# NLAFET/preAlps

Hardware: AMD Instinct MI355X
Metric: ECG iters/sec + SpMM HBM GB/s (% roofline), 3D-elasticity n~1M t=4 (higher is better)
Workload: dtype f64; 1 GPU; Q1 3-D elasticity, 70^3 nodes, the reference's element matrix (nu=0.25), stiff/soft inclusions (examples/test_ecg_petsc_ela.c:217-347) (N=1029000, nnz=80990208), ECG odir + block-Jacobi, t=4, tol 1e-5; nparts=5670, partition=boxes of [2, 4, 8] nodes, parallelism=rows x1, comm=none, hip_graphs=False, bj_max_bandwidth=35, spmm_blocks=4174

## Files before the change

### prealps_amd/csrc/bj_priv.h

```cpp
#ifndef PA_BJ_PRIV_H
#define PA_BJ_PRIV_H

#include "pa_host.h"
#include "bj_build.h"
#include "coarse_space.h"

typedef struct {
  int on;
  int k, naggr, nc, nchunks, n;
  double* V;
  int* part_aggregate;
  double* d_zv; int* d_ch_row0; int* d_ch_nrows; int* d_ch_aggr; int* d_agg_ptr; int* d_agg_chunk;
  double* d_Einv; double* d_partial; double* d_c; double* d_y;
  pa_coarse_plan_t plan;
  double bytes, setup_s;
  int builds; long long applies;
} pa_bj_coarse_t;

typedef struct {
  int created;
  pa_bj_coarse_t co;
  int np;
  int m;
  int* d_row0; int* d_nrows; int* d_bw; long long* d_off;
  int* d_map_f; int* d_map_b;
  double* d_Lf; double* d_Lb; double* d_invd_f; double* d_invd_b;
  double* d_Lf2; double* d_Lb2; long long* d_off2;
  double pairs_bytes;
  void* d_Lg4; int g4_bits; double g4_bytes;
  int* d_class_list[PA_BJ_MAX_CLASSES];
  const int* class_list_c[PA_BJ_MAX_CLASSES];
  pa_bj_plan_t plan;
  double factor_bytes; int nd_blocks;
  pa_bj_layout_t lay;
  int* h_row0; int* h_nrows; int* h_bw; int* h_grow0; int* h_map_f; char* h_is_nd;
  int row_off, dev_factor, dev_wmax, nd_bits;
  const int* A_rowptr;
  int op_build;
  unsigned* d_bm_src; unsigned* d_bm_dst; int* d_bm_chunk_blk; unsigned* d_bm_chunk_first;
  size_t bm_n, bm_nchunks, bm_bytes;
  long long* d_boff; int* d_slist; int* d_blist; int* d_fail;
  int bm_builds, updates, nd_rebuilt;
  double upd_map_s, upd_copy_s, upd_kernel_s, upd_total_s;
} pa_bj_t;

pa_bj_t* pa_bj_state(void);
void pa_bj_apply_epoch_bump(void);
void pa_bj_values_epoch_sync(void);
int pa_bj_factor_launch(const pa_bj_t* s, const int* d_slist, const int* d_blist, const long long* d_boff,
                        double* d_band, int* d_fail, int* fail);
int pa_bj_fail_global_row(int row_off, const int* map_f, const int* row0, const int* nrows, int np, int fail);
int pa_bj_nd_handoff(const char* who, const CPLM_Mat_CSR_t* A, int np, const char* is_nd, int nnd, const int* row0,
                     const int* nrows, const int* grow0, int m, int bits, int row_off);
int pa_bj_launch_g4(const pa_bj_t* s);
int pa_bj_launch_pairs(const pa_bj_t* s);

void pa_bj_coarse_release(pa_bj_coarse_t* co);
int pa_bj_coarse_refresh(pa_bj_t* s, const pa_operator_info_t* op);

#endif
```

### prealps_amd/csrc/bj_refactor.hip

```cpp
#include "kernels_common.h"

namespace {

__global__ __launch_bounds__(WG) void k_bj_band_assemble(const unsigned* __restrict__ src, const unsigned* __restrict__ dst,
                                                        const int* __restrict__ chunk_blk,
                                                        const unsigned* __restrict__ chunk_first, int nchunks,
                                                        const long long* __restrict__ boff,
                                                        const double* __restrict__ pv, double* __restrict__ band) {
  for (int c = blockIdx.x; c < nchunks; c += gridDim.x) {
    const unsigned e0 = chunk_first[c], e1 = chunk_first[c + 1];
    double* __restrict__ out = band + boff[chunk_blk[c]];
    for (unsigned base = e0 + threadIdx.x; base < e1; base += 4 * WG) {
      unsigned s[4], d[4];
      double v[4];
#pragma unroll
      for (int u = 0; u < 4; ++u) {
        const unsigned e = base + u * WG;
        s[u] = e < e1 ? __builtin_nontemporal_load(src + e) : 0u;
        d[u] = e < e1 ? __builtin_nontemporal_load(dst + e) : 0u;
      }
#pragma unroll
      for (int u = 0; u < 4; ++u) v[u] = base + u * WG < e1 ? pv[s[u]] : 0.0;
#pragma unroll
      for (int u = 0; u < 4; ++u) if (base + u * WG < e1) out[d[u]] = v[u];
    }
  }
}

}

extern "C" int pa_k_bj_band_assemble(const unsigned* src, const unsigned* dst, const int* chunk_blk,
                                     const unsigned* chunk_first, size_t nchunks, const long long* boff,
                                     const double* pv, double* band) {
  if (nchunks == 0) return 0;
  if (nchunks > 0x7fffffffu) { pa_rt_set_error("k_bj_band_assemble: %zu chunks", nchunks); return 1; }
  const int cus = pa_rt_num_cus() > 0 ? pa_rt_num_cus() : 256;
  size_t blocks = nchunks;
  if (blocks > (size_t)8 * cus) blocks = (size_t)8 * cus;
  PA_LAUNCH(k_bj_band_assemble, dim3((unsigned)blocks), dim3(WG), 0, cur_stream(), src, dst, chunk_blk, chunk_first,
            (int)nchunks, boff, pv, band);
  return kfail("k_bj_band_assemble");
}
```

### prealps_amd/csrc/bj_update.c

```c
#include <stdio.h>
#include <stdlib.h>
#include <string.h>

#include "bj_priv.h"

#define BJU_FAIL(...) pa_fail_at("preAlps_BlockJacobiUpdateValues", __VA_ARGS__)

static void bj_band_map_release(pa_bj_t* s) {
  pa_rt_free(s->d_bm_src); pa_rt_free(s->d_bm_dst); pa_rt_free(s->d_bm_chunk_blk); pa_rt_free(s->d_bm_chunk_first);
  pa_rt_free(s->d_boff); pa_rt_free(s->d_slist); pa_rt_free(s->d_blist); pa_rt_free(s->d_fail);
  s->d_bm_src = s->d_bm_dst = s->d_bm_chunk_first = NULL; s->d_bm_chunk_blk = s->d_slist = s->d_blist = s->d_fail = NULL;
  s->d_boff = NULL;
}

static int bj_ensure_band_map(pa_bj_t* s, const pa_operator_info_t* op) {
  if (s->d_bm_src) return 0;
  const int np = s->np;
  const pa_bj_layout_t* L = &s->lay;
  const double t0 = pa_wtime();
  pa_bj_band_map_in_t in = {.np = np, .rowPtr = op->A.rowPtr, .colInd = op->A.colInd, .row0 = s->h_row0, .nrows = s->h_nrows,
                            .grow0 = s->h_grow0, .bw = s->h_bw, .order = s->h_map_f, .is_nd = s->h_is_nd,
                            .wmax = s->dev_wmax, .chunk = 1024};
  pa_bj_band_map_t bm;
  const int brc = pa_bj_band_map_build(&in, &bm);
  if (brc == -2)
    return BJU_FAIL("the band of block %d (%d rows, bandwidth %d) has 2^32 entries or more: free and create instead",
                    bm.bad_block, s->h_nrows[bm.bad_block], s->h_bw[bm.bad_block]);
  if (brc == -3) return BJU_FAIL("block %d of the panel no longer has the pattern the preconditioner was created from", bm.bad_block);
  if (brc) return BJU_FAIL("out of host memory for the band map");
  ++s->bm_builds;
  int rc = 0;
  s->d_bm_src = (unsigned*)pa_rt_malloc((bm.n ? bm.n : 1) * sizeof(unsigned));
  s->d_bm_dst = (unsigned*)pa_rt_malloc((bm.n ? bm.n : 1) * sizeof(unsigned));
  s->d_bm_chunk_blk = (int*)pa_rt_malloc((bm.nchunks ? bm.nchunks : 1) * sizeof(int));
  s->d_bm_chunk_first = (unsigned*)pa_rt_malloc((bm.nchunks + 1) * sizeof(unsigned));
  s->d_boff = (long long*)pa_rt_malloc(((size_t)np + 1) * sizeof(long long));
  s->d_slist = (int*)pa_rt_malloc((L->ns ? L->ns : 1) * sizeof(int));
  s->d_blist = (int*)pa_rt_malloc((L->nbig ? L->nbig : 1) * sizeof(int));
  s->d_fail = (int*)pa_rt_malloc(sizeof(int));
  if (!s->d_bm_src || !s->d_bm_dst || !s->d_bm_chunk_blk || !s->d_bm_chunk_first || !s->d_boff || !s->d_slist ||
      !s->d_blist || !s->d_fail ||
      pa_rt_h2d(s->d_bm_src, bm.src, bm.n * sizeof(unsigned)) || pa_rt_h2d(s->d_bm_dst, bm.dst, bm.n * sizeof(unsigned)) ||
      pa_rt_h2d(s->d_bm_chunk_blk, bm.chunk_blk, bm.nchunks * sizeof(int)) ||
      pa_rt_h2d(s->d_bm_chunk_first, bm.chunk_first, (bm.nchunks + 1) * sizeof(unsigned)) ||
      pa_rt_h2d(s->d_boff, L->boff, ((size_t)np + 1) * sizeof(long long)) ||
      pa_rt_h2d(s->d_slist, L->slist, (size_t)L->ns * sizeof(int)) || pa_rt_h2d(s->d_blist, L->blist, (size_t)L->nbig * sizeof(int))) {
    rc = BJU_FAIL("uploading the band map (%zu entries) failed: %s", bm.n, pa_rt_error());
    bj_band_map_release(s);
  }
  if (!rc) {
    s->bm_n = bm.n; s->bm_nchunks = bm.nchunks; s->bm_bytes = pa_bj_band_map_bytes(&bm);
    s->upd_map_s = pa_wtime() - t0;
  }
  pa_bj_band_map_free(&bm);
  return rc;
}

static int bj_refactor_bands(pa_bj_t* s, const pa_operator_info_t* op, int* wrote, int* spd_fail) {
  const size_t lnnz = (size_t)op->A.rowPtr[s->m], btot = s->lay.btot;
  double* d_pv = (double*)pa_rt_malloc((lnnz ? lnnz : 1) * sizeof(double));
  double* d_band = (double*)pa_rt_malloc((btot ? btot : 1) * sizeof(double));
  void* e0 = pa_rt_event_create();
  void* e1 = pa_rt_event_create();
  int rc = 0, fail = 0;
  if (!d_pv || !d_band || !e0 || !e1)
    rc = BJU_FAIL("no device memory for the panel values (%zu) and the bands (%zu entries): %s", lnnz, btot, pa_rt_error());
  if (!rc) {
    const double t0 = pa_wtime();
    if (pa_rt_h2d(d_pv, op->A.val, lnnz * sizeof(double))) rc = BJU_FAIL("uploading the panel values failed: %s", pa_rt_error());
    s->upd_copy_s = pa_wtime() - t0;
  }
  if (!rc) {
    *wrote = 1;
    if (pa_rt_event_record(e0) || pa_rt_memset(d_band, 0, btot * sizeof(double)) || pa_rt_memset(s->d_fail, 0, sizeof(int)) ||
        pa_k_bj_band_assemble(s->d_bm_src, s->d_bm_dst, s->d_bm_chunk_blk, s->d_bm_chunk_first, s->bm_nchunks, s->d_boff,
                              d_pv, d_band) ||
        pa_bj_factor_launch(s, s->d_slist, s->d_blist, s->d_boff, d_band, s->d_fail, &fail))
      rc = BJU_FAIL("factorising the diagonal blocks on the device failed: %s", pa_rt_error());
    *spd_fail = fail;
  }
  if (!rc && fail == 0) {
    if (s->d_Lg4 && pa_bj_launch_g4(s)) rc = BJU_FAIL("k_bj_g4_setup failed");
    if (!rc && s->d_Lf2 && pa_bj_launch_pairs(s)) rc = BJU_FAIL("k_bj_pairs failed");
    if (!rc && (pa_rt_event_record(e1) || pa_rt_sync())) rc = BJU_FAIL("%s", pa_rt_error());
    if (!rc) s->upd_kernel_s = pa_rt_event_elapsed_s(e0, e1);
  }
  pa_rt_event_destroy(e0); pa_rt_event_destroy(e1);
  pa_rt_free(d_pv); pa_rt_free(d_band);
  return rc;
}

int preAlps_BlockJacobiUpdateValues(void) {
  pa_bj_t* s = pa_bj_state();
  const double t_all = pa_wtime();
  if (!s->created) return BJU_FAIL("preconditioner not created");
  const pa_operator_info_t* op = pa_operator_info();
  if (!op) return BJU_FAIL("operator not built: it was freed since preAlps_BlockJacobiCreate (free and create instead)");
  if (pa_operator_build_count() != s->op_build)
    return BJU_FAIL("the operator was built again since preAlps_BlockJacobiCreate: free and create instead");
  if (s->A_rowptr != op->A.rowPtr)
    return BJU_FAIL("the preconditioner was not created from the operator's own panel (preAlps_OperatorGetA): free and create instead");
  if (!s->dev_factor)
    return BJU_FAIL("the preconditioner was created with PREALPS_BJ_FACTOR=host, its records come from the host "
                    "Cholesky: free and create instead");
  int rc = 0, wrote = 0, spd_fail = 0;
  s->upd_copy_s = s->upd_kernel_s = 0.0;
  if (s->np - s->nd_blocks > 0) {
    rc = bj_ensure_band_map(s, op);
    if (rc) return rc;
    rc = bj_refactor_bands(s, op, &wrote, &spd_fail);
    if (!rc && spd_fail > 0)
      rc = BJU_FAIL("diagonal block is not SPD (global row %d)",
                    pa_bj_fail_global_row(s->row_off, s->h_map_f, s->h_row0, s->h_nrows, s->np, spd_fail));
    if (rc && !wrote) return rc;
  }
  if (!rc && s->nd_blocks > 0) {
    rc = pa_bj_nd_handoff("preAlps_BlockJacobiUpdateValues", &op->A, s->np, s->h_is_nd, s->nd_blocks, s->h_row0, s->h_nrows,
                          s->h_grow0, s->m, s->nd_bits, s->row_off);
    if (!rc) { s->nd_rebuilt = s->nd_blocks; s->factor_bytes = 2.0 * 8.0 * (double)s->lay.tot + pa_nd_factor_bytes(); }
  }
  if (rc) { preAlps_BlockJacobiFree(); return rc; }
  ++s->updates;
  pa_bj_values_epoch_sync();
  if (s->co.on) rc = pa_bj_coarse_refresh(s, op);
  s->upd_total_s = pa_wtime() - t_all;
  return rc;
}

int pa_bj_update_stat(const char* key, double* value) {
  const pa_bj_t* s = pa_bj_state();
  const int on = s->created;
  if (!strcmp(key, "bj_updates")) *value = on ? s->updates : 0;
  else if (!strcmp(key, "bj_update_nd_rebuilt")) *value = on ? s->nd_rebuilt : 0;
  else if (!strcmp(key, "bj_band_map_builds")) *value = on ? s->bm_builds : 0;
  else if (!strcmp(key, "bj_band_map_entries")) *value = on && s->d_bm_src ? (double)s->bm_n : 0.0;
  else if (!strcmp(key, "bj_band_map_bytes")) *value = on && s->d_bm_src ? (double)s->bm_bytes : 0.0;
  else if (!strcmp(key, "bj_update_map_s")) *value = on ? s->upd_map_s : 0.0;
  else if (!strcmp(key, "bj_update_copy_s")) *value = on ? s->upd_copy_s : 0.0;
  else if (!strcmp(key, "bj_update_kernel_s")) *value = on ? s->upd_kernel_s : 0.0;
  else if (!strcmp(key, "bj_update_total_s")) *value = on ? s->upd_total_s : 0.0;
  else if (!strcmp(key, "bj_records_address")) *value = on ? (double)(size_t)s->d_Lf : 0.0;
  else if (!strcmp(key, "bj_g4_address")) *value = on ? (double)(size_t)s->d_Lg4 : 0.0;
  else if (!strcmp(key, "bj_coarse_max_dofs")) *value = PA_COARSE_MAX_DOFS;
  else if (!strncmp(key, "bj_coarse_", 10)) {
    const pa_bj_coarse_t* co = &s->co;
    const int con = on && co->on;
    const char* sub = key + 10;
    if (!strcmp(sub, "dofs")) *value = con ? co->nc : 0;
    else if (!strcmp(sub, "vectors")) *value = con ? co->k : 0;
    else if (!strcmp(sub, "aggregates")) *value = con ? co->naggr : 0;
    else if (!strcmp(sub, "chunks")) *value = con ? co->nchunks : 0;
    else if (!strcmp(sub, "bytes")) *value = con ? co->bytes : 0.0;
    else if (!strcmp(sub, "setup_s")) *value = con ? co->setup_s : 0.0;
    else if (!strcmp(sub, "builds")) *value = con ? co->builds : 0;
    else if (!strcmp(sub, "applies")) *value = con ? (double)co->applies : 0.0;
    else if (!strcmp(sub, "einv_address")) *value = con ? (double)(size_t)co->d_Einv : 0.0;
    else return 1;
  }
  else return 1;
  return 0;
}
```

### prealps_amd/csrc/block_jacobi.c

```c
#include <stdio.h>
#include <stdlib.h>
#include <string.h>

#include "bj_priv.h"

static pa_bj_t g_bj;
pa_bj_t* pa_bj_state(void) { return &g_bj; }
static double g_bj_setup_s[2];
double pa_bj_setup_seconds(int which) { return g_bj_setup_s[which ? 1 : 0]; }

double pa_bj_factor_bytes(void) { return g_bj.created ? g_bj.factor_bytes : 0.0; }
static int g_bj_values_epoch;
int pa_bj_values_epoch(void) { return g_bj_values_epoch; }
void pa_bj_values_epoch_sync(void) { g_bj_values_epoch = pa_operator_values_epoch(); }
int pa_bj_max_bandwidth(void) { return g_bj.created ? g_bj.lay.max_bw : 0; }
int pa_bj_nparts(void) { return g_bj.created ? g_bj.np : 0; }
int pa_bj_nd_blocks(void) { return g_bj.created ? g_bj.nd_blocks : 0; }
int pa_bj_nd_precision(void) { return g_bj.created && g_bj.nd_blocks > 0 ? pa_nd_precision() : 0; }

static int g_nd_bits = 0;
int preAlps_hip_set_nd_precision(int bits) {
  if (bits != 0 && bits != 32 && bits != 64)
    return PA_FAIL("precision %d refused: 64 (double), 32 (single) or 0 (follow PREALPS_BJ_ND_PRECISION)", bits);
  g_nd_bits = bits;
  return 0;
}
int pa_bj_band_precision(void) { return g_bj.created && g_bj.d_Lg4 ? g_bj.g4_bits : 0; }

static int g_band_bits = 0;
int preAlps_hip_set_band_precision(int bits) {
  if (bits != 0 && bits != 32 && bits != 64)
    return PA_FAIL("precision %d refused: 64 (double), 32 (single) or 0 (follow PREALPS_BJ_BAND_PRECISION)", bits);
  g_band_bits = bits;
  return 0;
}
double pa_bj_pairs_bytes(void) { return g_bj.created ? g_bj.pairs_bytes : 0.0; }
double pa_bj_g4_bytes(void) { return g_bj.created ? g_bj.g4_bytes : 0.0; }
int pa_bj_gram_blocks(void) {
  const pa_bj_t* s = &g_bj;
  const pa_bj_layout_t* L = &s->lay;
  if (!s->created || s->nd_blocks > 0 || !s->d_Lg4 || L->nclass != 1 || !L->class_g4[0] || L->class_count[0] != s->np) return 0;
  if (s->co.on) return 0;
  return s->np;
}

static int g_bj_apply_epoch;
int pa_bj_apply_epoch(void) { return g_bj_apply_epoch; }
void pa_bj_apply_epoch_bump(void) { ++g_bj_apply_epoch; }

void preAlps_BlockJacobiFree(void) {
  pa_bj_t* s = &g_bj;
  pa_bj_coarse_release(&s->co);
  ++g_bj_apply_epoch;
  pa_rt_free(s->d_row0); pa_rt_free(s->d_nrows); pa_rt_free(s->d_bw); pa_rt_free(s->d_off);
  pa_rt_free(s->d_map_f); pa_rt_free(s->d_map_b);
  pa_rt_free(s->d_Lf); pa_rt_free(s->d_Lb); pa_rt_free(s->d_invd_f); pa_rt_free(s->d_invd_b);
  pa_rt_free(s->d_Lf2); pa_rt_free(s->d_Lb2); pa_rt_free(s->d_off2); pa_rt_free(s->d_Lg4);
  for (int c = 0; c < PA_BJ_MAX_CLASSES; ++c) pa_rt_free(s->d_class_list[c]);
  pa_bj_layout_free(&s->lay);
  free(s->h_row0); free(s->h_nrows); free(s->h_bw); free(s->h_grow0); free(s->h_map_f); free(s->h_is_nd);
  pa_rt_free(s->d_bm_src); pa_rt_free(s->d_bm_dst); pa_rt_free(s->d_bm_chunk_blk); pa_rt_free(s->d_bm_chunk_first);
  pa_rt_free(s->d_boff); pa_rt_free(s->d_slist); pa_rt_free(s->d_blist); pa_rt_free(s->d_fail);
  pa_nd_free();
  memset(s, 0, sizeof(*s));
}

#define BJ_FAIL(...) pa_fail_at("preAlps_BlockJacobiCreate", __VA_ARGS__)

typedef struct {
  int nd_bits, band_bits;
  int nd_mode, nd_rows;
  int dev_factor;
  int wide_from;
  int want_g4, want_pairs;
} bj_switches_t;

static int bj_storage_bits(int set, const char* name, const char* what, int* bits) {
  const char* pe = getenv(name);
  if (set) *bits = set;
  else if (!pe || !*pe || !strcmp(pe, "double")) *bits = 64;
  else if (!strcmp(pe, "single")) *bits = 32;
  else return BJ_FAIL("%s=%s: expected double or single (storage of the %s)", name, pe, what);
  return 0;
}

static int bj_read_switches(bj_switches_t* sw) {
  if (bj_storage_bits(g_nd_bits, "PREALPS_BJ_ND_PRECISION", "sparse block factors", &sw->nd_bits) ||
      bj_storage_bits(g_band_bits, "PREALPS_BJ_BAND_PRECISION", "one-copy band records", &sw->band_bits))
    return 1;
  sw->nd_mode = getenv("PREALPS_BJ_ND") ? atoi(getenv("PREALPS_BJ_ND")) : 1;
  sw->nd_rows = getenv("PREALPS_BJ_ND_ROWS") ? atoi(getenv("PREALPS_BJ_ND_ROWS")) : 2048;
  const char* fenv = getenv("PREALPS_BJ_FACTOR");
  sw->dev_factor = !(fenv && !strcmp(fenv, "host"));
  const char* e = getenv("PREALPS_BJ_WIDE_FROM");
  sw->wide_from = -1;
  if (e && *e) { sw->wide_from = atoi(e); if (sw->wide_from < 0) sw->wide_from = 0; }
  sw->want_g4 = !(getenv("PREALPS_BJ_G4") && atoi(getenv("PREALPS_BJ_G4")) == 0);
  sw->want_pairs = !(getenv("PREALPS_BJ_PAIRS") && atoi(getenv("PREALPS_BJ_PAIRS")) == 0);
  return 0;
}

static int bj_alloc_records(pa_bj_t* s) {
  const size_t m = (size_t)s->m, tot = s->lay.tot, pad = s->lay.pad;
  s->d_invd_f = (double*)pa_rt_malloc((m ? m : 1) * sizeof(double));
  s->d_invd_b = (double*)pa_rt_malloc((m ? m : 1) * sizeof(double));
  s->d_Lf = (double*)pa_rt_malloc((tot + pad) * sizeof(double));
  s->d_Lb = (double*)pa_rt_malloc((tot + pad) * sizeof(double));
  if (!s->d_Lf || !s->d_Lb || !s->d_invd_f || !s->d_invd_b ||
      pa_rt_memset(s->d_Lf, 0, (tot + pad) * sizeof(double)) || pa_rt_memset(s->d_Lb, 0, (tot + pad) * sizeof(double)))
    return BJ_FAIL("allocating %zu factor entries on the device failed: %s", tot, pa_rt_error());
  return 0;
}

static int bj_layout_host(pa_bj_t* s, pa_bj_build_t* B) {
  const int np = B->np;
  const pa_bj_layout_t* L = &s->lay;
  const long long* off = L->off;
  const size_t cap = (size_t)32 << 20;
  size_t sf_cap = 0;
  double* sf = NULL; double* sg = NULL;
  int rc = 0, q = 0;
  while (L->ndev + L->nnd < np && q < np && !rc) {
    if (s->dev_factor || B->is_nd[q]) { ++q; continue; }
    int q1 = q;
    while (q1 < np && !s->dev_factor && !B->is_nd[q1] && (q1 == q || (size_t)(off[q1 + 1] - off[q]) <= cap)) ++q1;
    size_t len = (size_t)(off[q1] - off[q]);
    if (len > sf_cap) {
      sf_cap = len;
      sf = (double*)realloc(sf, sf_cap * sizeof(double));
      sg = (double*)realloc(sg, sf_cap * sizeof(double));
      if (!sf || !sg) { rc = BJ_FAIL("out of host memory for %zu factor entries", sf_cap); break; }
    }
    memset(sf, 0, len * sizeof(double));
    memset(sg, 0, len * sizeof(double));
    int nitem = 0;
    for (int x = q; x < q1; ++x) nitem += (B->nrows[x] + 255) / 256;
    int* item_part = (int*)malloc((nitem ? nitem : 1) * sizeof(int));
    int* item_j0 = (int*)malloc((nitem ? nitem : 1) * sizeof(int));
    if (!item_part || !item_j0) { free(item_part); free(item_j0); rc = BJ_FAIL("out of host memory for %d slabs", nitem); break; }
    nitem = 0;
    for (int x = q; x < q1; ++x)
      for (int j0 = 0; j0 < B->nrows[x]; j0 += 256) { item_part[nitem] = x; item_j0[nitem++] = j0; }
#pragma omp parallel for num_threads(pa_host_threads()) schedule(dynamic, 4)
    for (int it = 0; it < nitem; ++it) {
      const int x = item_part[it];
      pa_bj_layout_slab(B, L->wide_from, x, item_j0[it], sf + (off[x] - off[q]), sg + (off[x] - off[q]));
    }
    free(item_part); free(item_j0);
    if (pa_rt_h2d(s->d_Lf + off[q], sf, len * sizeof(double)) || pa_rt_h2d(s->d_Lb + off[q], sg, len * sizeof(double)))
      rc = BJ_FAIL("uploading the block factors failed: %s", pa_rt_error());
    q = q1;
  }
  free(sf); free(sg);
  if (!rc && (pa_rt_h2d(s->d_invd_f, B->invd_f, (size_t)B->m * sizeof(double)) ||
              pa_rt_h2d(s->d_invd_b, B->invd_b, (size_t)B->m * sizeof(double))))
    rc = BJ_FAIL("uploading the block factors failed: %s", pa_rt_error());
  return rc;
}

static int bj_upload_classes(pa_bj_t* s) {
  const pa_bj_layout_t* L = &s->lay;
  int rc = 0;
  for (int c = 0; c < L->nclass && !rc; ++c) {
    const size_t bytes = (size_t)L->class_count[c] * sizeof(int);
    s->d_class_list[c] = (int*)pa_rt_malloc(bytes);
    rc = !s->d_class_list[c] || pa_rt_h2d(s->d_class_list[c], L->class_list[c], bytes);
    s->class_list_c[c] = s->d_class_list[c];
  }
  if (rc) rc = BJ_FAIL("uploading block lists failed: %s", pa_rt_error());
  return rc;
}

static int bj_upload_index(pa_bj_t* s, const pa_bj_build_t* B) {
  const int np = B->np, m = B->m;
  s->d_row0 = (int*)pa_rt_malloc(np * sizeof(int));
  s->d_nrows = (int*)pa_rt_malloc(np * sizeof(int));
  s->d_bw = (int*)pa_rt_malloc(np * sizeof(int));
  s->d_off = (long long*)pa_rt_malloc((np + 1) * sizeof(long long));
  s->d_map_f = (int*)pa_rt_malloc((size_t)(m ? m : 1) * sizeof(int));
  s->d_map_b = (int*)pa_rt_malloc((size_t)(m ? m : 1) * sizeof(int));
  int bad = !s->d_row0 || !s->d_nrows || !s->d_bw || !s->d_off || !s->d_map_f || !s->d_map_b;
  bad = bad || pa_rt_h2d(s->d_row0, B->row0, np * sizeof(int)) || pa_rt_h2d(s->d_nrows, B->nrows, np * sizeof(int)) ||
// ... 95 lines not shown
                   pa_bj_fail_global_row(s->row_off, B->map_f, B->row0, B->nrows, np, fail));
  }
  if (tr) fprintf(stderr, "[setup] device factorisation + layout  %.3f s\n", pa_wtime() - t_tr);
  pa_rt_free(d_band); pa_rt_free(d_boff); pa_rt_free(d_slist); pa_rt_free(d_blist); pa_rt_free(d_fail);
  return rc;
}

int pa_bj_nd_handoff(const char* who, const CPLM_Mat_CSR_t* A, int np, const char* is_nd, int nnd, const int* row0,
                     const int* nrows, const int* grow0, int m, int bits, int row_off) {
  int* ndl = (int*)malloc((size_t)(nnd ? nnd : 1) * sizeof(int));
  int x = 0, nd_fail = -1, rc = 0;
  if (!ndl) return pa_fail_at(who, "out of host memory");
  for (int q = 0; q < np; ++q) if (is_nd[q]) ndl[x++] = q;
  const int r2 = pa_nd_create(A, nnd, ndl, row0, nrows, grow0, m, bits, &nd_fail);
  if (r2 == 2) rc = pa_fail_at(who, "diagonal block is not SPD (global row %d)", row_off + nd_fail);
  else if (r2) rc = 1;
  free(ndl);
  return rc;
}

int pa_bj_launch_g4(const pa_bj_t* s) {
  const pa_bj_layout_t* L = &s->lay;
  for (int c = 0; c < L->nclass; ++c)
    if (L->class_g4[c] &&
        (s->g4_bits == 32
           ? pa_k_bj_g4_setup_f32(s->d_class_list[c], L->class_count[c], s->d_nrows, s->d_bw, s->d_off, s->d_off2, s->d_Lf, (float*)s->d_Lg4)
           : pa_k_bj_g4_setup(s->d_class_list[c], L->class_count[c], s->d_nrows, s->d_bw, s->d_off, s->d_off2, s->d_Lf, (double*)s->d_Lg4)))
      return 1;
  return 0;
}

int pa_bj_launch_pairs(const pa_bj_t* s) {
  const pa_bj_layout_t* L = &s->lay;
  for (int c = 0; c < L->nclass; ++c)
    if (L->class_pairs[c])
      if (pa_k_bj_pairs(s->d_class_list[c], L->class_count[c], s->d_nrows, s->d_bw, s->d_off, s->d_off2, s->d_Lf, s->d_Lf2) ||
          pa_k_bj_pairs(s->d_class_list[c], L->class_count[c], s->d_nrows, s->d_bw, s->d_off, s->d_off2, s->d_Lb, s->d_Lb2))
        return 1;
  return 0;
}

static int bj_make_g4(pa_bj_t* s, int band_bits) {
  const long long tot2 = s->lay.tot2;
  const size_t esz = band_bits == 32 ? sizeof(float) : sizeof(double);
  const size_t g4_alloc = (size_t)tot2 * esz + 8192;
  s->g4_bits = band_bits;
  s->d_Lg4 = pa_rt_malloc(g4_alloc);
  if (!s->d_Lg4 || pa_rt_memset(s->d_Lg4, 0, g4_alloc))
    return BJ_FAIL("allocating the one-copy sweep records failed: %s", pa_rt_error());
  if (pa_bj_launch_g4(s)) return BJ_FAIL("k_bj_g4_setup failed");
  s->g4_bytes = (double)esz * (double)tot2;
  return 0;
}

static int bj_make_pairs(pa_bj_t* s) {
  const long long tot2 = s->lay.tot2;
  s->d_Lf2 = (double*)pa_rt_malloc(((size_t)tot2 + 1024) * sizeof(double));
  s->d_Lb2 = (double*)pa_rt_malloc(((size_t)tot2 + 1024) * sizeof(double));
  if (!s->d_Lf2 || !s->d_Lb2 ||
      pa_rt_memset(s->d_Lf2 + tot2, 0, 512 * sizeof(double)) || pa_rt_memset(s->d_Lb2 + tot2, 0, 512 * sizeof(double)))
    return BJ_FAIL("allocating the paired sweep records failed: %s", pa_rt_error());
  if (pa_bj_launch_pairs(s)) return BJ_FAIL("k_bj_pairs failed");
  s->pairs_bytes = 2.0 * 8.0 * (double)tot2;
  return 0;
}

static int bj_second_layouts(pa_bj_t* s, int band_bits) {
  const pa_bj_layout_t* L = &s->lay;
  const size_t np1 = (size_t)s->np + 1;
  int rc = 0;
  if (!L->any_g4 && !L->any_pairs) return 0;
  s->d_off2 = (long long*)pa_rt_malloc(np1 * sizeof(long long));
  if (!s->d_off2 || pa_rt_h2d(s->d_off2, L->off2, np1 * sizeof(long long)))
    rc = BJ_FAIL("allocating the second sweep records failed: %s", pa_rt_error());
  if (!rc && L->any_g4) rc = bj_make_g4(s, band_bits);
  if (!rc && L->any_pairs) rc = bj_make_pairs(s);
  if (!rc && pa_rt_sync()) rc = BJ_FAIL("%s", pa_rt_error());
  return rc;
}

static void bj_fill_plan(pa_bj_t* s) {
  pa_bj_plan_t* pl = &s->plan;
  const pa_bj_layout_t* L = &s->lay;
  pl->nparts = s->np; pl->row0 = s->d_row0; pl->nrows = s->d_nrows; pl->bw = s->d_bw; pl->off = s->d_off;
  pl->map_f = s->d_map_f; pl->map_b = s->d_map_b; pl->Lf = s->d_Lf; pl->Lb = s->d_Lb;
  pl->invd_f = s->d_invd_f; pl->invd_b = s->d_invd_b;
  pl->Lf2 = s->d_Lf2; pl->Lb2 = s->d_Lb2; pl->off2 = s->d_off2;
  pl->Lg4 = s->d_Lg4; pl->g4_bits = s->d_Lg4 ? s->g4_bits : 0; pl->class_g4 = L->class_g4; pl->class_bmax = L->class_bmax;
  pl->nclass = L->nclass; pl->class_R = L->class_R; pl->class_count = L->class_count;
  pl->class_wmax = L->class_wmax;
  pl->class_list = s->class_list_c;
}

static void* bj_dup(const void* p, size_t bytes) {
  void* c = malloc(bytes ? bytes : 1);
  if (c) memcpy(c, p, bytes);
  return c;
}

static int bj_keep_decisions(pa_bj_t* s, const pa_bj_build_t* B, const pa_bj_build_in_t* in) {
  const size_t np = (size_t)B->np;
  s->h_row0 = (int*)bj_dup(B->row0, np * sizeof(int));
  s->h_nrows = (int*)bj_dup(B->nrows, np * sizeof(int));
  s->h_bw = (int*)bj_dup(B->bw, np * sizeof(int));
  s->h_is_nd = (char*)bj_dup(B->is_nd, np);
  s->h_map_f = (int*)bj_dup(B->map_f, (size_t)B->m * sizeof(int));
  s->h_grow0 = (int*)bj_dup(in->grow, np * sizeof(int));
  if (!s->h_row0 || !s->h_nrows || !s->h_bw || !s->h_is_nd || !s->h_map_f || !s->h_grow0)
    return BJ_FAIL("out of host memory for the block arrays");
  s->A_rowptr = in->rowPtr; s->op_build = pa_operator_build_count();
  return 0;
}

int preAlps_BlockJacobiCreate(CPLM_Mat_CSR_t* A, int* rowPos, int sizeRowPos, int* colPos,
                              int sizeColPos) {
  (void)colPos; (void)sizeColPos;
  PA_REQUIRE_GPU();
  const pa_operator_info_t* op = pa_operator_info();
  if (!op) return PA_FAIL("the operator must be built before the preconditioner");
  if (!A || !A->rowPtr || !rowPos || sizeRowPos != op->nparts + 1)
    return PA_FAIL(" wrong test 'A != NULL && sizeRowPos == nparts + 1'");
  bj_switches_t sw;
  if (bj_read_switches(&sw)) return 1;
  if (g_bj.created) preAlps_BlockJacobiFree();
  pa_bj_t* s = &g_bj;
  const pa_bj_build_in_t in = {.np = op->part1 - op->part0, .m = op->m, .rowPtr = A->rowPtr, .colInd = A->colInd, .val = A->val,
                               .grow = rowPos + op->part0, .row_off = op->row_off, .nd_mode = sw.nd_mode, .nd_rows = sw.nd_rows,
                               .dev_factor = sw.dev_factor, .dev_wmax = pa_bj_factor_wmax(), .threads = pa_host_threads()};
  s->np = in.np; s->m = in.m;
  s->row_off = in.row_off; s->dev_factor = in.dev_factor; s->dev_wmax = in.dev_wmax; s->nd_bits = sw.nd_bits;

  double t_setup0 = pa_wtime();
  pa_bj_build_t B;
  int rc = pa_bj_build_blocks(&in, &B);
  g_bj_setup_s[0] = pa_wtime() - t_setup0;
  t_setup0 = pa_wtime();
  if (rc == PA_BJ_NOT_SPD) rc = BJ_FAIL("diagonal block is not SPD (global row %d)", B.fail_row);
  else if (rc && B.nomem_block >= 0) rc = BJ_FAIL("out of host memory for block %d", B.nomem_block);
  else if (rc) rc = BJ_FAIL("out of host memory for the block arrays");
  if (!rc) {
    const pa_bj_layout_in_t lin = {.np = in.np, .nrows = B.nrows, .bw = B.bw, .is_nd = B.is_nd, .factor_wmax = in.dev_wmax,
                                   .max_R = pa_bj_max_R(), .g4_max_band = pa_bj_g4_max_band(), .g4_max_rows = pa_bj_g4_max_rows(),
                                   .dev_factor = in.dev_factor, .wide_from = sw.wide_from,
                                   .want_g4 = sw.want_g4 && (long long)in.m * 16 < 2147483647LL, .want_pairs = sw.want_pairs};
    char err[256];
    const int lrc = pa_bj_layout_build(&lin, &s->lay, err, sizeof(err));
    if (lrc == PA_BJ_BANDWIDTH) rc = BJ_FAIL("%s", err);
    else if (lrc) rc = BJ_FAIL("out of host memory for the layout of %d blocks", in.np);
  }
  if (!rc) rc = bj_alloc_records(s);
  if (!rc) rc = bj_layout_host(s, &B);
  if (!rc) rc = bj_upload_classes(s);
  if (!rc) rc = bj_upload_index(s, &B);
  if (!rc && s->lay.ndev > 0) rc = bj_factor_device(s, &B);
  if (!rc && s->lay.nnd > 0)
    rc = pa_bj_nd_handoff("preAlps_BlockJacobiCreate", A, in.np, B.is_nd, s->lay.nnd, B.row0, B.nrows, in.grow, in.m, sw.nd_bits,
                          in.row_off);
  if (!rc) rc = bj_second_layouts(s, sw.band_bits);
  if (!rc) rc = bj_keep_decisions(s, &B, &in);
  pa_bj_build_free(&B);
  if (rc) { preAlps_BlockJacobiFree(); return rc; }
  s->factor_bytes = 2.0 * 8.0 * (double)s->lay.tot + pa_nd_factor_bytes();
  s->nd_blocks = s->lay.nnd;
  bj_fill_plan(s);
  s->created = 1;
  ++g_bj_apply_epoch;
  pa_bj_values_epoch_sync();
  g_bj_setup_s[1] = pa_wtime() - t_setup0;
  return 0;
}

int preAlps_BlockJacobiApply(CPLM_Mat_Dense_t* A_in, CPLM_Mat_Dense_t* B_out) {
  pa_bj_t* s = &g_bj;
  if (!s->created) return PA_FAIL("preconditioner not created");
  if (!A_in || !B_out || !A_in->val || !B_out->val) return PA_FAIL(" wrong test 'A_in->val != NULL && B_out->val != NULL'");
  int ts = pa_desc_stride(A_in);
  if (pa_desc_stride(B_out) != ts || A_in->info.m != s->m)
    return PA_FAIL("panel shapes do not match the preconditioner (m %d vs %d)", A_in->info.m, s->m);
  B_out->info.n = A_in->info.n; B_out->info.N = A_in->info.N;
  B_out->info.nval = B_out->info.m * B_out->info.n;
  pa_time_begin(PA_T_PRECOND);
  if (s->co.on) pa_k_bj_gram_disarm(NULL);
  if (pa_k_bj_apply(&s->plan, ts, A_in->val, B_out->val)) return PA_FAIL("block-Jacobi kernel launch failed: %s", pa_rt_error());
  if (s->nd_blocks > 0 && pa_nd_apply(ts, A_in->val, B_out->val)) return 1;
  if (s->co.on && A_in->info.n > 0) {
    if (pa_k_coarse_apply(&s->co.plan, ts, A_in->info.n, A_in->val, B_out->val)) return PA_FAIL("coarse correction failed: %s", pa_rt_error());
    ++s->co.applies;
  }
  pa_time_end(PA_T_PRECOND);
  return 0;
}

int preAlps_PreconditionerCreate(PreAlps_preconditioner_t** precond, Prec_Type_t precond_type, void* data) {
  if (!precond) return PA_FAIL(" wrong test 'precond != NULL'");
  *precond = (PreAlps_preconditioner_t*)malloc(sizeof(PreAlps_preconditioner_t));
  if (!*precond) return PA_FAIL("Malloc fails for precond[].");
  (*precond)->side = LEFT_PREC;
  (*precond)->type = precond_type;
  (*precond)->data = data;
  return 0;
}

int preAlps_PreconditionerDestroy(PreAlps_preconditioner_t** precond) {
  if (precond && *precond) { free(*precond); *precond = NULL; }
  return 0;
}

int preAlps_PreconditionerMatApply(PreAlps_preconditioner_t* precond, CPLM_Mat_Dense_t* A_in,
                                   CPLM_Mat_Dense_t* B_out) {
  if (!precond) return PA_FAIL(" wrong test 'precond != NULL'");
  if (precond->type == PREALPS_BLOCKJACOBI) return preAlps_BlockJacobiApply(A_in, B_out);
  if (precond->type == PREALPS_NOPREC) {
    if (!A_in || !B_out || !A_in->val || !B_out->val) return PA_FAIL(" wrong test 'A_in->val != NULL && B_out->val != NULL'");
    int ts = pa_desc_stride(A_in);
    if (pa_desc_stride(B_out) != ts || A_in->info.m != B_out->info.m)
      return PA_FAIL("panel shapes do not match (m %d vs %d)", A_in->info.m, B_out->info.m);
    B_out->info.n = A_in->info.n; B_out->info.N = A_in->info.N;
    B_out->info.nval = B_out->info.m * B_out->info.n;
    if (pa_rt_d2d(B_out->val, A_in->val, (size_t)A_in->info.m * ts * sizeof(double))) return PA_FAIL("%s", pa_rt_error());
    return 0;
  }
  return PA_FAIL("Unknown preconditioner: %d (LORASC / PRESC are not part of this library)", (int)precond->type);
}
```

### prealps_amd/csrc/pa_device.h

```cpp
#ifndef PA_DEVICE_H
#define PA_DEVICE_H
#include <stddef.h>
#ifdef __cplusplus
extern "C" {
#endif

int pa_rt_init(int device);
void pa_rt_shutdown(void);
int pa_rt_ready(void);
void pa_rt_set_stream(void* s);
void* pa_rt_stream(void);
int pa_rt_sync(void);
const char* pa_rt_error(void);
void pa_rt_set_error(const char* fmt, ...) __attribute__((format(printf, 1, 2)));
void* pa_rt_malloc(size_t bytes);
void pa_rt_free(void* d);
void* pa_rt_host_alloc(size_t bytes);
void* pa_rt_host_alloc_coherent(size_t bytes);
int pa_rt_stream_state(void);
void pa_rt_host_free(void* h);
int pa_rt_memset(void* d, int v, size_t bytes);
int pa_rt_h2d(void* d, const void* h, size_t bytes);
int pa_rt_d2h(void* h, const void* d, size_t bytes);
int pa_rt_d2d(void* dst, const void* src, size_t bytes);
// ... 123 lines not shown
double pa_k_take_note_seq(const double* host);
int pa_k_copy_cols(int m, int ts, int nc, const double* src, double* dst);
int pa_k_right_mult(int m, int ts, int t, const double* Q, double* A);
int pa_k_permute_trsm(int m, int ts, int n, const int* piv, int t, const double* U, const double* src, double* dst);
int pa_k_permute_cols(int m, int ts, int n, const int* piv, double* A);
int pa_k_rowsum(int m, int ts, int nc, const double* X, double* sol);
int pa_k_multi_start(int m, int ts, int k, int s, const double* B, int ldb, const int* pcol, double* R,
                     double* sums, int* nblk);
int pa_k_guess_split(int m, int ts, int k, int s, const double* X0, int ld, const int* pcol, double* X);
int pa_k_guess_start(int m, int ts, int k, int s, const double* B, int ldb, const int* pcol, const double* AX,
                     double* R, double* bsums, double* rsums, int* nblk);
int pa_k_group_norms(const double* rtr_partials, int nblk, int ts, int k, int s, double* out, double* host);
int pa_k_group_norms_ride(const double* rtr_partials, int nblk, int ts, int k, int s, const int* info, double* buf);
int pa_k_rowsum_groups(int m, int ts, int k, int s, const double* X, double* sol, int ld);
int pa_k_sys_gather(int m, int ts, int k, const int* src, const double* dl, const double* B, int ldb, const double* X0,
                    int ldx0, double* Bp, double* X0p, double* sums, int* nblk);
int pa_k_sys_scatter(int m, int ts, int k, int s, const double* X, const int* src, const double* dl, double* Xout,
                     int ldx);
int pa_k_sys_norms(int m, int ts, int k, int s, const double* R, const double* dl, double* part, int* nblk);
int pa_k_sys_copy_rows(int m, int k, const int* src, const double* Xin, int ldin, double* Xout, int ldout);
int pa_k_sys_norms_ride(const double* rtr_part, int rtr_nblk, const double* sys_part, int sys_nblk, int ts, int k, int s,
                        const int* info, double* buf);

typedef struct {
  int nparts;
  const int* row0;
  const int* nrows;
  const int* bw;
  const long long* off;
  const int* map_f;
  const int* map_b;
  const double* Lf;
  const double* Lb;
  const double* Lf2; const double* Lb2; const long long* off2;
  const void* Lg4;
  int g4_bits;
  const int* class_g4;
  const int* class_bmax;
  const double* invd_f;
  const double* invd_b;
  int nclass;
  const int* class_R;
  const int* class_count;
  const int* class_wmax;
  const int* const* class_list;
} pa_bj_plan_t;
#ifdef __HIPCC__
#define PA_HOST_DEVICE __host__ __device__
#else
#define PA_HOST_DEVICE
#endif
static inline PA_HOST_DEVICE int pa_bj_wide_window(int w) {
  int W = (w + 64 + 63) & ~63;
  if (W <= 1024) return W;
  W = (w + 64 + 127) & ~127;
  if (W <= 2048) return W;
  return (w + 64 + 255) & ~255;
}
int pa_k_bj_g4(const pa_bj_plan_t* pl, const int* list, int count, int wmax, int bmax, int xs, int ncol,
                const double* in, double* out);
void pa_k_bj_g4_gram(const double* prev, double* part);
int pa_bj_max_R(void);
int pa_k_bj_pairs(const int* list, int count, const int* nrows, const int* bw, const long long* off,
                  const long long* off2, const double* L, double* L2);
int pa_bj_g4_max_rows(void);
int pa_bj_g4_max_band(void);
int pa_bj_g4_max_band8(void);
int pa_k_bj_g4_setup(const int* list, int count, const int* nrows, const int* bw, const long long* off,
                      const long long* off2, const double* L, double* Lg4);
int pa_k_bj_g4_setup_f32(const int* list, int count, const int* nrows, const int* bw, const long long* off,
                          const long long* off2, const double* L, float* Lg4);
int pa_bj_g4_last(int which);
int pa_bj_factor_wmax(void);
int pa_k_scatter(size_t n, const long long* off, const double* val, double* dst);
int pa_k_bj_factor_big(const int* list, int count, int wmax, int wide_from, const int* row0, const int* nrows,
                       const int* bw, const long long* off, const long long* boff, double* band, double* Lf, double* Lb,
                       double* invd_f, double* invd_b, int* fail);
int pa_k_bj_factor(const int* list, int count, int wmax, const int* row0, const int* nrows, const int* bw,
                   const long long* off, const long long* boff, const double* band, double* Lf, double* Lb,
                   double* invd_f, double* invd_b, int* fail);
int pa_k_bj_apply(const pa_bj_plan_t* pl, int ts, const double* in, double* out);
int pa_k_bj_band_assemble(const unsigned* src, const unsigned* dst, const int* chunk_blk, const unsigned* chunk_first,
                          size_t nchunks, const long long* boff, const double* pv, double* band);

typedef struct {
  int m, k, naggr, nc, nchunks;
  const double* zv;
  const int* ch_row0; const int* ch_nrows; const int* ch_aggr;
  const int* agg_ptr; const int* agg_chunk;
  const double* Einv;
  double* partial; double* c; double* y;
} pa_coarse_plan_t;
int pa_k_coarse_apply(const pa_coarse_plan_t* pl, int ts, int ncols, const double* in, double* out);

#define PA_ND_LD(x) (((x) + 15) & ~15)
typedef struct {
  const int* n; const int* m; const int* ld; const long long* offF; const long long* offB; const int* rows_off;
  const int* coff; const int* ccoff; const int* rows; const int* src; const double* dinv;
  const double* F; const double* B; double* contrib; double* Y;
  const float* F32; const float* B32;
  int nlevel;
  const int* f_count; const int* const* f_front; const int* const* f_row0;
  const int* b_count; const int* const* b_front; const int* const* b_col0;
} pa_nd_plan_t;
typedef struct {
  const int* n; const int* m; const int* ld; const long long* offF; const long long* offB; const int* rows_off;
  const int* rows; const int* src; const int* child; const int* newrow;
  const long long* acol0; const long long* acp; const int* ari; const double* acv;
  const unsigned long long* front; const int* ldf;
  double* F; double* B; double* dinv; unsigned long long* fail;
} pa_ndf_args_t;
int pa_k_ndf_assemble(const pa_ndf_args_t* a, const int* tf, const int* ti, const int* tj, int ntiles,
                      const int* fronts, int nfronts);
int pa_k_ndf_potrf(const pa_ndf_args_t* a, const int* fronts, int nfronts, int jb);
int pa_k_ndf_trsm(const pa_ndf_args_t* a, const int* cfront, const int* crow0, int nchunks, int jb, int inverse);
int pa_k_ndf_update(const pa_ndf_args_t* a, const int* tf, const int* ti, const int* tj, int ntiles, int jb,
                    int inverse);
int pa_k_ndf_pinit(const pa_ndf_args_t* a, const int* cfront, const int* crow0, int nchunks);
int pa_k_ndf_finalize(const pa_ndf_args_t* a, const int* tf, const int* ti, const int* tj, int ntiles);
int pa_k_ndf_check(const pa_ndf_args_t* a, const int* fronts, int nfronts, int nmax);

int pa_nd_chunk_rows(void);
int pa_nd_block_cols(void);
int pa_k_nd_apply(const pa_nd_plan_t* pl, int ts, const double* in, double* out);
int pa_k_nd_round(const double* src, float* dst, size_t n);

#ifdef __cplusplus
}
#endif
#endif
```

Baseline: 3428 iterations/s.

## Share factor storage reads across block-Jacobi blocks with identical bands

At setup, diagonal blocks are hashed and compared byte-for-byte so that blocks with identical band matrices map to one representative. The apply plan then reads factors through per-block offsets pointing at that representative, so repeated factors hit the same memory and cache, which cuts HBM traffic during block-Jacobi apply. On value updates a GPU kernel rechecks whether each member still equals its representative and falls back to its own factor when it differs. This adds host hashing at setup, a check kernel and a readback on every update, and exploits duplicated blocks in regular meshes.

Result: faster. 4083 iterations/s (median of 6 runs) (+19.1%).

```diff
diff --git a/prealps_amd/csrc/bj_priv.h b/prealps_amd/csrc/bj_priv.h
--- a/prealps_amd/csrc/bj_priv.h
+++ b/prealps_amd/csrc/bj_priv.h
@@ -3,6 +3,7 @@
 
 #include "pa_host.h"
 #include "bj_build.h"
+#include "bj_share.h"
 #include "coarse_space.h"
 
 typedef struct {
@@ -27,6 +28,11 @@
   double* d_Lf; double* d_Lb; double* d_invd_f; double* d_invd_b;
   double* d_Lf2; double* d_Lb2; long long* d_off2;
   double pairs_bytes;
+  long long* d_off_read; long long* d_off2_read;
+  int* d_rep; int* d_share_list; unsigned long long* d_share_cnt;
+  int share_on, share_classes, share_members, shared_blocks;
+  long long shared_elems2;
+  double share_s;
   void* d_Lg4; int g4_bits; double g4_bytes;
   int* d_class_list[PA_BJ_MAX_CLASSES];
   const int* class_list_c[PA_BJ_MAX_CLASSES];
@@ -34,6 +40,7 @@
   double factor_bytes; int nd_blocks;
   pa_bj_layout_t lay;
   int* h_row0; int* h_nrows; int* h_bw; int* h_grow0; int* h_map_f; char* h_is_nd;
+  int* h_rep;
   int row_off, dev_factor, dev_wmax, nd_bits;
   const int* A_rowptr;
   int op_build;
diff --git a/prealps_amd/csrc/bj_refactor.hip b/prealps_amd/csrc/bj_refactor.hip
--- a/prealps_amd/csrc/bj_refactor.hip
+++ b/prealps_amd/csrc/bj_refactor.hip
@@ -27,6 +27,40 @@
   }
 }
 
+__global__ __launch_bounds__(WG) void k_bj_share_check(const int* __restrict__ list, const int* __restrict__ rep,
+                                                      const int* __restrict__ nrows, const int* __restrict__ bw,
+                                                      const long long* __restrict__ boff, const double* __restrict__ band,
+                                                      const long long* __restrict__ off, const long long* __restrict__ off2,
+                                                      long long* __restrict__ off_read, long long* __restrict__ off2_read,
+                                                      unsigned long long* __restrict__ cnt) {
+  const int p = list[blockIdx.x], r = rep[p];
+  const int b = nrows[p], w = bw[p];
+  const size_t n = (size_t)b * (size_t)(w + 1);
+  const unsigned long long* __restrict__ x = reinterpret_cast<const unsigned long long*>(band + boff[p]);
+  const unsigned long long* __restrict__ y = reinterpret_cast<const unsigned long long*>(band + boff[r]);
+  int differ = 0;
+  for (size_t i = threadIdx.x; i < n; i += WG) differ |= x[i] != y[i];
+  differ = __syncthreads_or(differ);
+  if (threadIdx.x == 0) {
+    const int from = differ ? p : r;
+    off_read[p] = off[from];
+    if (off2_read) off2_read[p] = off2[from];
+    if (!differ) {
+      atomicAdd(&cnt[0], 1ull);
+      atomicAdd(&cnt[1], (unsigned long long)(8 * ((b + 7) / 8)) * (unsigned long long)(w + 4));
+    }
+  }
+}
+
+}
+
+extern "C" int pa_k_bj_share_check(const int* list, int count, const int* rep, const int* nrows, const int* bw,
+                                   const long long* boff, const double* band, const long long* off, const long long* off2,
+                                   long long* off_read, long long* off2_read, unsigned long long* cnt) {
+  if (count <= 0) return 0;
+  PA_LAUNCH(k_bj_share_check, dim3((unsigned)count), dim3(WG), 0, cur_stream(), list, rep, nrows, bw, boff, band, off, off2,
+            off_read, off2_read, cnt);
+  return kfail("k_bj_share_check");
 }
 
 extern "C" int pa_k_bj_band_assemble(const unsigned* src, const unsigned* dst, const int* chunk_blk,
diff --git a/prealps_amd/csrc/bj_share.c b/prealps_amd/csrc/bj_share.c
--- /dev/null
+++ b/prealps_amd/csrc/bj_share.c
@@ -0,0 +1,65 @@
+#include <stdlib.h>
+#include <string.h>
+
+#include "bj_share.h"
+
+typedef struct { unsigned long long h; int nrows, bw, p; } share_key_t;
+
+static unsigned long long band_hash(const double* band, size_t n) {
+  unsigned long long h = 0x9E3779B97F4A7C15ull ^ (unsigned long long)n;
+  for (size_t i = 0; i < n; ++i) {
+    unsigned long long x;
+    memcpy(&x, band + i, sizeof(x));
+    h = (h ^ x) * 0xFF51AFD7ED558CCDull;
+    h ^= h >> 29;
+  }
+  return h;
+}
+
+static int key_cmp(const void* a, const void* b) {
+  const share_key_t* x = (const share_key_t*)a;
+  const share_key_t* y = (const share_key_t*)b;
+  if (x->h != y->h) return x->h < y->h ? -1 : 1;
+  if (x->nrows != y->nrows) return x->nrows < y->nrows ? -1 : 1;
+  if (x->bw != y->bw) return x->bw < y->bw ? -1 : 1;
+  return x->p < y->p ? -1 : (x->p > y->p ? 1 : 0);
+}
+
+static size_t band_bytes(const share_key_t* k) { return (size_t)k->nrows * ((size_t)k->bw + 1) * sizeof(double); }
+
+int pa_bj_share_classes(const pa_bj_share_in_t* in, int* rep, int* nclass) {
+  const int np = in->np, threads = in->threads > 0 ? in->threads : 1;
+  int ne = 0;
+  for (int p = 0; p < np; ++p) { rep[p] = p; ne += in->eligible[p] && in->bands[p]; }
+  *nclass = np;
+  if (ne < 2) return 0;
+  share_key_t* key = (share_key_t*)malloc((size_t)ne * sizeof(share_key_t));
+  int* first = (int*)malloc((size_t)ne * sizeof(int));
+  int* reps = (int*)malloc((size_t)ne * sizeof(int));
+  char* same = (char*)malloc((size_t)ne);
+  if (!key || !first || !reps || !same) { free(key); free(first); free(reps); free(same); return -1; }
+  ne = 0;
+  for (int p = 0; p < np; ++p)
+    if (in->eligible[p] && in->bands[p]) { key[ne].nrows = in->nrows[p]; key[ne].bw = in->bw[p]; key[ne].p = p; ++ne; }
+#pragma omp parallel for num_threads(threads) schedule(dynamic, 16)
+  for (int i = 0; i < ne; ++i)
+    key[i].h = band_hash(in->bands[key[i].p], (size_t)key[i].nrows * ((size_t)key[i].bw + 1)) & in->hash_mask;
+  qsort(key, (size_t)ne, sizeof(share_key_t), key_cmp);
+  for (int i = 0; i < ne; ++i)
+    first[i] = i > 0 && key[i].h == key[i - 1].h && key[i].nrows == key[i - 1].nrows && key[i].bw == key[i - 1].bw ? first[i - 1] : i;
+#pragma omp parallel for num_threads(threads) schedule(dynamic, 16)
+  for (int i = 0; i < ne; ++i)
+    same[i] = first[i] != i && !memcmp(in->bands[key[i].p], in->bands[key[first[i]].p], band_bytes(&key[i]));
+  int nreps = 0, shared = 0;
+  for (int i = 0; i < ne; ++i) {
+    if (first[i] == i) { nreps = 0; reps[nreps++] = key[i].p; continue; }
+    int r = same[i] ? reps[0] : -1;
+    for (int k = 1; k < nreps && r < 0; ++k)
+      if (!memcmp(in->bands[key[i].p], in->bands[reps[k]], band_bytes(&key[i]))) r = reps[k];
+    if (r < 0) reps[nreps++] = key[i].p;
+    else { rep[key[i].p] = r; ++shared; }
+  }
+  *nclass = np - shared;
+  free(key); free(first); free(reps); free(same);
+  return 0;
+}
diff --git a/prealps_amd/csrc/bj_share.h b/prealps_amd/csrc/bj_share.h
--- /dev/null
+++ b/prealps_amd/csrc/bj_share.h
@@ -0,0 +1,17 @@
+#ifndef PA_BJ_SHARE_H
+#define PA_BJ_SHARE_H
+
+#include <stddef.h>
+
+typedef struct {
+  int np;
+  const int* nrows; const int* bw;
+  const char* eligible;
+  double* const* bands;
+  int threads;
+  unsigned long long hash_mask;
+} pa_bj_share_in_t;
+
+int pa_bj_share_classes(const pa_bj_share_in_t* in, int* rep, int* nclass);
+
+#endif
diff --git a/prealps_amd/csrc/bj_update.c b/prealps_amd/csrc/bj_update.c
--- a/prealps_amd/csrc/bj_update.c
+++ b/prealps_amd/csrc/bj_update.c
@@ -75,9 +75,18 @@
     if (pa_rt_event_record(e0) || pa_rt_memset(d_band, 0, btot * sizeof(double)) || pa_rt_memset(s->d_fail, 0, sizeof(int)) ||
         pa_k_bj_band_assemble(s->d_bm_src, s->d_bm_dst, s->d_bm_chunk_blk, s->d_bm_chunk_first, s->bm_nchunks, s->d_boff,
                               d_pv, d_band) ||
+        (s->share_members > 0 &&
+         (pa_rt_memset(s->d_share_cnt, 0, 2 * sizeof(unsigned long long)) ||
+          pa_k_bj_share_check(s->d_share_list, s->share_members, s->d_rep, s->d_nrows, s->d_bw, s->d_boff, d_band, s->d_off,
+                              s->d_off2, s->d_off_read, s->d_off2_read, s->d_share_cnt))) ||
         pa_bj_factor_launch(s, s->d_slist, s->d_blist, s->d_boff, d_band, s->d_fail, &fail))
       rc = BJU_FAIL("factorising the diagonal blocks on the device failed: %s", pa_rt_error());
     *spd_fail = fail;
+    if (!rc && s->share_members > 0) {
+      unsigned long long cnt[2];
+      if (pa_rt_d2h(cnt, s->d_share_cnt, sizeof(cnt))) rc = BJU_FAIL("%s", pa_rt_error());
+      else { s->shared_blocks = (int)cnt[0]; s->shared_elems2 = (long long)cnt[1]; }
+    }
   }
   if (!rc && fail == 0) {
     if (s->d_Lg4 && pa_bj_launch_g4(s)) rc = BJU_FAIL("k_bj_g4_setup failed");
@@ -139,6 +148,11 @@
   else if (!strcmp(key, "bj_update_copy_s")) *value = on ? s->upd_copy_s : 0.0;
   else if (!strcmp(key, "bj_update_kernel_s")) *value = on ? s->upd_kernel_s : 0.0;
   else if (!strcmp(key, "bj_update_total_s")) *value = on ? s->upd_total_s : 0.0;
+  else if (!strcmp(key, "bj_share_classes")) *value = on ? s->share_classes : 0;
+  else if (!strcmp(key, "bj_shared_blocks")) *value = on ? s->shared_blocks : 0;
+  else if (!strcmp(key, "bj_share_distinct_g4_bytes"))
+    *value = on && s->d_Lg4 ? (s->g4_bits == 32 ? 4.0 : 8.0) * (double)(s->lay.tot2 - s->shared_elems2) : 0.0;
+  else if (!strcmp(key, "bj_share_s")) *value = on ? s->share_s : 0.0;
   else if (!strcmp(key, "bj_records_address")) *value = on ? (double)(size_t)s->d_Lf : 0.0;
   else if (!strcmp(key, "bj_g4_address")) *value = on ? (double)(size_t)s->d_Lg4 : 0.0;
   else if (!strcmp(key, "bj_coarse_max_dofs")) *value = PA_COARSE_MAX_DOFS;
diff --git a/prealps_amd/csrc/block_jacobi.c b/prealps_amd/csrc/block_jacobi.c
--- a/prealps_amd/csrc/block_jacobi.c
+++ b/prealps_amd/csrc/block_jacobi.c
@@ -56,6 +56,8 @@
   pa_rt_free(s->d_map_f); pa_rt_free(s->d_map_b);
   pa_rt_free(s->d_Lf); pa_rt_free(s->d_Lb); pa_rt_free(s->d_invd_f); pa_rt_free(s->d_invd_b);
   pa_rt_free(s->d_Lf2); pa_rt_free(s->d_Lb2); pa_rt_free(s->d_off2); pa_rt_free(s->d_Lg4);
+  pa_rt_free(s->d_off_read); pa_rt_free(s->d_off2_read); pa_rt_free(s->d_rep); pa_rt_free(s->d_share_list); pa_rt_free(s->d_share_cnt);
+  free(s->h_rep);
   for (int c = 0; c < PA_BJ_MAX_CLASSES; ++c) pa_rt_free(s->d_class_list[c]);
   pa_bj_layout_free(&s->lay);
   free(s->h_row0); free(s->h_nrows); free(s->h_bw); free(s->h_grow0); free(s->h_map_f); free(s->h_is_nd);
@@ -73,6 +75,7 @@
   int dev_factor;
   int wide_from;
   int want_g4, want_pairs;
+  int share;
 } bj_switches_t;
 
 static int bj_storage_bits(int set, const char* name, const char* what, int* bits) {
@@ -97,7 +100,58 @@
   if (e && *e) { sw->wide_from = atoi(e); if (sw->wide_from < 0) sw->wide_from = 0; }
   sw->want_g4 = !(getenv("PREALPS_BJ_G4") && atoi(getenv("PREALPS_BJ_G4")) == 0);
   sw->want_pairs = !(getenv("PREALPS_BJ_PAIRS") && atoi(getenv("PREALPS_BJ_PAIRS")) == 0);
-  return 0;
+  sw->share = !(getenv("PREALPS_BJ_SHARE") && atoi(getenv("PREALPS_BJ_SHARE")) == 0);
+  return 0;
+}
+
+static int bj_share_pass(pa_bj_t* s, const pa_bj_build_t* B, int share) {
+  const int np = B->np;
+  const double t0 = pa_wtime();
+  s->h_rep = (int*)malloc((size_t)(np ? np : 1) * sizeof(int));
+  char* el = (char*)malloc((size_t)(np ? np : 1));
+  if (!s->h_rep || !el) { free(el); return BJ_FAIL("out of host memory for the classes of %d blocks", np); }
+  for (int p = 0; p < np; ++p) el[p] = share && !B->is_nd[p] && B->bands[p] && B->bw[p] <= s->lay.wide_from;
+  const pa_bj_share_in_t in = {.np = np, .nrows = B->nrows, .bw = B->bw, .eligible = el, .bands = B->bands,
+                               .threads = pa_host_threads(), .hash_mask = ~0ull};
+  const int rc = pa_bj_share_classes(&in, s->h_rep, &s->share_classes);
+  free(el);
+  if (rc) return BJ_FAIL("out of host memory for the classes of %d blocks", np);
+  s->share_on = share; s->share_members = 0; s->shared_elems2 = 0;
+  for (int p = 0; p < np; ++p)
+    if (s->h_rep[p] != p) { ++s->share_members; s->shared_elems2 += 8LL * ((B->nrows[p] + 7) / 8) * (B->bw[p] + 4); }
+  s->shared_blocks = s->share_members;
+  s->share_s = pa_wtime() - t0;
+  if (getenv("PREALPS_SETUP_TRACE"))
+    fprintf(stderr, "[setup] block classes (%d of %d blocks share, %d classes)  %.3f s\n", s->share_members, np,
+            s->share_classes, s->share_s);
+  return 0;
+}
+
+static int bj_upload_share(pa_bj_t* s) {
+  const int np = s->np, nm = s->share_members;
+  const size_t np1 = (size_t)np + 1;
+  const pa_bj_layout_t* L = &s->lay;
+  long long* h = (long long*)malloc(2 * np1 * sizeof(long long));
+  int* list = (int*)malloc((size_t)(nm ? nm : 1) * sizeof(int));
+  int rc = 0, x = 0;
+  if (!h || !list) { free(h); free(list); return BJ_FAIL("out of host memory for the read offsets of %d blocks", np); }
+  for (int p = 0; p < np; ++p) {
+    h[p] = L->off[s->h_rep[p]]; h[np1 + p] = L->off2[s->h_rep[p]];
+    if (s->h_rep[p] != p) list[x++] = p;
+  }
+  h[np] = L->off[np]; h[np1 + np] = L->off2[np];
+  s->d_off_read = (long long*)pa_rt_malloc(np1 * sizeof(long long));
+  if (s->d_off2) s->d_off2_read = (long long*)pa_rt_malloc(np1 * sizeof(long long));
+  s->d_rep = (int*)pa_rt_malloc((size_t)(np ? np : 1) * sizeof(int));
+  s->d_share_list = (int*)pa_rt_malloc((size_t)(nm ? nm : 1) * sizeof(int));
+  s->d_share_cnt = (unsigned long long*)pa_rt_malloc(2 * sizeof(unsigned long long));
+  if (!s->d_off_read || (s->d_off2 && !s->d_off2_read) || !s->d_rep || !s->d_share_list || !s->d_share_cnt ||
+      pa_rt_h2d(s->d_off_read, h, np1 * sizeof(long long)) ||
+      (s->d_off2 && pa_rt_h2d(s->d_off2_read, h + np1, np1 * sizeof(long long))) ||
+      pa_rt_h2d(s->d_rep, s->h_rep, (size_t)np * sizeof(int)) || pa_rt_h2d(s->d_share_list, list, (size_t)nm * sizeof(int)))
+    rc = BJ_FAIL("uploading the read offsets failed: %s", pa_rt_error());
+  free(h); free(list);
+  return rc;
 }
 
 static int bj_alloc_records(pa_bj_t* s) {
@@ -359,10 +413,10 @@
 static void bj_fill_plan(pa_bj_t* s) {
   pa_bj_plan_t* pl = &s->plan;
   const pa_bj_layout_t* L = &s->lay;
-  pl->nparts = s->np; pl->row0 = s->d_row0; pl->nrows = s->d_nrows; pl->bw = s->d_bw; pl->off = s->d_off;
+  pl->nparts = s->np; pl->row0 = s->d_row0; pl->nrows = s->d_nrows; pl->bw = s->d_bw; pl->off = s->d_off_read;
   pl->map_f = s->d_map_f; pl->map_b = s->d_map_b; pl->Lf = s->d_Lf; pl->Lb = s->d_Lb;
   pl->invd_f = s->d_invd_f; pl->invd_b = s->d_invd_b;
-  pl->Lf2 = s->d_Lf2; pl->Lb2 = s->d_Lb2; pl->off2 = s->d_off2;
+  pl->Lf2 = s->d_Lf2; pl->Lb2 = s->d_Lb2; pl->off2 = s->d_off2_read;
   pl->Lg4 = s->d_Lg4; pl->g4_bits = s->d_Lg4 ? s->g4_bits : 0; pl->class_g4 = L->class_g4; pl->class_bmax = L->class_bmax;
   pl->nclass = L->nclass; pl->class_R = L->class_R; pl->class_count = L->class_count;
   pl->class_wmax = L->class_wmax;
@@ -425,6 +479,7 @@
     if (lrc == PA_BJ_BANDWIDTH) rc = BJ_FAIL("%s", err);
     else if (lrc) rc = BJ_FAIL("out of host memory for the layout of %d blocks", in.np);
   }
+  if (!rc) rc = bj_share_pass(s, &B, sw.share);
   if (!rc) rc = bj_alloc_records(s);
   if (!rc) rc = bj_layout_host(s, &B);
   if (!rc) rc = bj_upload_classes(s);
@@ -434,6 +489,7 @@
     rc = pa_bj_nd_handoff("preAlps_BlockJacobiCreate", A, in.np, B.is_nd, s->lay.nnd, B.row0, B.nrows, in.grow, in.m, sw.nd_bits,
                           in.row_off);
   if (!rc) rc = bj_second_layouts(s, sw.band_bits);
+  if (!rc) rc = bj_upload_share(s);
   if (!rc) rc = bj_keep_decisions(s, &B, &in);
   pa_bj_build_free(&B);
   if (rc) { preAlps_BlockJacobiFree(); return rc; }
diff --git a/prealps_amd/csrc/pa_device.h b/prealps_amd/csrc/pa_device.h
--- a/prealps_amd/csrc/pa_device.h
+++ b/prealps_amd/csrc/pa_device.h
@@ -229,6 +229,9 @@
 int pa_k_bj_apply(const pa_bj_plan_t* pl, int ts, const double* in, double* out);
 int pa_k_bj_band_assemble(const unsigned* src, const unsigned* dst, const int* chunk_blk, const unsigned* chunk_first,
                           size_t nchunks, const long long* boff, const double* pv, double* band);
+int pa_k_bj_share_check(const int* list, int count, const int* rep, const int* nrows, const int* bw, const long long* boff,
+                        const double* band, const long long* off, const long long* off2, long long* off_read,
+                        long long* off2_read, unsigned long long* cnt);
 
 typedef struct {
   int m, k, naggr, nc, nchunks;
```
